# HaoruXue/spline-trajectory-optimization

Hardware: AMD Instinct MI355X
Metric: min-curvature QP solves/sec (N=2000 waypoints) (higher is better)
Workload: dtype f64

## Files before the change

### spline_trajectory_optimization_amd/csrc/rl_device.hpp

```cpp
#pragma once
#include <hip/hip_runtime.h>


namespace rl {

constexpr int kWave = 64;
constexpr int kMaxK = 5;

struct TrackDev {
  int k, n, nt, N;
  const double* t;
  const double* c0;
  const int* ell;
  const double* D;
  const int* sup;
  const double* base;
  const double* Ds;
  const double* base_s;
};

template <int K>
__device__ __forceinline__ void deboor(const double* __restrict__ t, double x, int l, int m,
                                       double (&h)[K + 1]) {
  double hh[K + 1];
// ... 321 lines not shown
__device__ __forceinline__ int stage_prefetch(const double2* ring, int nr, int nchunk, bool active, int hint, double2* stg, int lane) {
  const unsigned long long m = __ballot(active && hint >= 0 && hint < nr);
  const int first = m ? __ffsll((long long)m) - 1 : 0;
  const int lo = __builtin_amdgcn_readlane(window_start(hint, nchunk), first);
  const int base = m ? lo : 0;
  asm volatile("s_waitcnt lgkmcnt(0)" ::: "memory");
  stage_issue(ring, nr, base, stg, lane);
  return base;
}

template <bool ST = false, typename RingPtr>
__device__ __forceinline__ Hit search_ring_brute(RingPtr ring, int nr, double px, double py,
                                                 double dx, double dy) {
  Hit h{INFINITY, 0.0, kNoEdge};
  scan_edges<ST>(ring, nr, 0, nr, px, py, dx, dy, h);
  return h;
}


template <bool ST = false, typename RingPtr, typename CirclePtr>
__device__ __forceinline__ Hit search_ring_culled(RingPtr ring, int nr, CirclePtr circ, int nchunk,
                                                  double px, double py, double dx, double dy,
                                                  double dlen) {
  Hit h{INFINITY, 0.0, kNoEdge};
  for (int c = 0; c < nchunk; ++c) {
    const double mx = circ[3 * c] - px, my = circ[3 * c + 1] - py, r = circ[3 * c + 2];
    const double rr = r * dlen * (1.0 + 1e-9) + 1e-9;
    if (fabs(mx * dy - my * dx) > rr) continue;
    if (fabs(mx * dx + my * dy) > (dlen + r) * dlen * (1.0 + 1e-9) + 1e-9) continue;
    const int j0 = c * kChunk;
    scan_edges<ST>(ring, nr, j0, min(kChunk, nr - j0), px, py, dx, dy, h);
  }
  return h;
}

template <int CTRL, int ROW_MASK>
__device__ __forceinline__ double dpp_mov(double identity, double v) {
  int lo = __double2loint(v), hi = __double2hiint(v);
  lo = __builtin_amdgcn_update_dpp(__double2loint(identity), lo, CTRL, ROW_MASK, 0xf, false);
  hi = __builtin_amdgcn_update_dpp(__double2hiint(identity), hi, CTRL, ROW_MASK, 0xf, false);
  return __hiloint2double(hi, lo);
}
struct OpSum { static __device__ __forceinline__ double id() { return 0.0; }
               static __device__ __forceinline__ double f(double a, double b) { return a + b; } };
struct OpMax { static __device__ __forceinline__ double id() { return -INFINITY; }
               static __device__ __forceinline__ double f(double a, double b) { return fmax(a, b); } };
struct OpMin { static __device__ __forceinline__ double id() { return INFINITY; }
               static __device__ __forceinline__ double f(double a, double b) { return fmin(a, b); } };

template <typename Op>
__device__ __forceinline__ double wave_reduce(double v) {
  const double e = Op::id();
  v = Op::f(v, dpp_mov<0x111, 0xf>(e, v));
  v = Op::f(v, dpp_mov<0x112, 0xf>(e, v));
  v = Op::f(v, dpp_mov<0x114, 0xf>(e, v));
  v = Op::f(v, dpp_mov<0x118, 0xf>(e, v));
  v = Op::f(v, dpp_mov<0x142, 0xa>(e, v));
  v = Op::f(v, dpp_mov<0x143, 0xc>(e, v));
  const int lo = __builtin_amdgcn_readlane(__double2loint(v), 63);
  const int hi = __builtin_amdgcn_readlane(__double2hiint(v), 63);
  return __hiloint2double(hi, lo);
}
template <typename Op>
__device__ __forceinline__ double wave_reduce_bfly(double v) {
#define RL_BFLY(pattern)                                                                                        \
  {                                                                                                             \
    const int lo_ = __builtin_amdgcn_ds_swizzle(__double2loint(v), pattern);                                    \
    const int hi_ = __builtin_amdgcn_ds_swizzle(__double2hiint(v), pattern);                                    \
    v = Op::f(v, __hiloint2double(hi_, lo_));                                                                   \
  }
  RL_BFLY(0x041F) RL_BFLY(0x081F) RL_BFLY(0x101F) RL_BFLY(0x201F) RL_BFLY(0x401F)
#undef RL_BFLY
  const int other = (((int)threadIdx.x ^ 32) & 63) << 2;
  const int lo_ = __builtin_amdgcn_ds_bpermute(other, __double2loint(v));
  const int hi_ = __builtin_amdgcn_ds_bpermute(other, __double2hiint(v));
  return Op::f(v, __hiloint2double(hi_, lo_));
}
__device__ __forceinline__ double wave_max_bfly(double v) { return wave_reduce_bfly<OpMax>(v); }
__device__ __forceinline__ double wave_min_bfly(double v) { return wave_reduce_bfly<OpMin>(v); }
__device__ __forceinline__ double wave_sum(double v) { return wave_reduce<OpSum>(v); }
__device__ __forceinline__ double wave_max(double v) { return wave_reduce<OpMax>(v); }
__device__ __forceinline__ double wave_min(double v) { return wave_reduce<OpMin>(v); }

template <bool STAGED = false, bool ST = false, typename RingPtr, typename CirclePtr>
__device__ __forceinline__ Hit search_ring_windowed(RingPtr ring, int nr, CirclePtr circ,
                                                    CirclePtr sep, int nchunk, bool active, int hint,
                                                    double px, double py, double dx, double dy,
                                                    double dlen, const double* cmax, bool skip_guard = false,
                                                    unsigned long long* stamps = nullptr,
                                                    double2* stg = nullptr, int staged_base = -1) {
  const int lane = threadIdx.x & (kWave - 1);
  Hit h{INFINITY, 0.0, kNoEdge};
  const bool windowed = active && hint >= 0 && hint < nr;
  const int lo = window_start(hint, nchunk);
#ifdef RL_STAMPS
  unsigned long long w0 = 0, w1 = 0;
  asm volatile("s_memtime %0\n\ts_waitcnt lgkmcnt(0)" : "=s"(w0) :: "memory");
#endif
  if constexpr (!STAGED) {
    if (windowed) scan_window<kWinBatch, ST>(ring, nr, lo, lo, px, py, dx, dy, h, cmax);
  } else {
    bool todo = windowed;
    int base = staged_base;
    if (base >= 0) stage_wait();
    for (;;) {
      if (base >= 0) {
        int off = lo - base;
        if (off < 0) off += nr;
        if (todo && (off & (kChunk - 1)) == 0 && off + kWinEdges + 1 <= kStage) {
          scan_window<kStageBatch, ST>(StagedWindow{stg + stage_slot(off)}, nr, 0, lo, px, py, dx, dy, h, cmax, stamps);
          todo = false;
        }
      }
      const unsigned long long left = __ballot(todo);
      if (left == 0ull) break;
      base = __builtin_amdgcn_readlane(lo, __ffsll((long long)left) - 1);
      asm volatile("s_waitcnt lgkmcnt(0)" ::: "memory");
      stage_issue(reinterpret_cast<const double2*>(ring), nr, base, stg, lane);
      stage_wait();
    }
  }
#ifdef RL_STAMPS
  asm volatile("s_waitcnt vmcnt(0)\n\ts_memtime %0\n\ts_waitcnt lgkmcnt(0)" : "=s"(w1) :: "memory");
  if (stamps) stamps[0] += w1 - w0;
#endif
  if (skip_guard) return h;
  const bool found = h.best <= 1.0;
  const double di = active ? ((found ? h.best * dlen : dlen) * (1.0 + 1e-9) + 1e-9) : 0.0;
  auto chunk_in_window = [&](int c) {
    const int e0 = c * kChunk;
    const int cnt = min(kChunk, nr - e0);
    int off = e0 - lo;
    if (off < 0) off += nr;
    return off + cnt - 1 <= kWinEdges - 1;
  };
  bool slow = active;
  if (windowed && found && nchunk > 2 * kNear + 1) {
    const int ce = h.edge / kChunk;
    bool ok = sep[ce] > 2.0 * di;
    const bool centred = ce * kChunk == lo + kChunk && lo + kWinEdges <= nr;
    if (ok && !centred) {
#pragma unroll
      for (int u = -kNear; u <= kNear; ++u) {
        int c = ce + u;
        if (c < 0) c += nchunk;
        if (c >= nchunk) c -= nchunk;
        if (!chunk_in_window(c)) {
          const double mx = circ[3 * c] - px, my = circ[3 * c + 1] - py;
          const double lim = (di + circ[3 * c + 2]) * (1.0 + 1e-9);
          ok = ok && !(mx * mx + my * my <= lim * lim);
        }
      }
    }
    slow = !ok;
  }
  const unsigned long long sm = __ballot(slow);
  if (sm == 0ull) return h;
  const int first = __ffsll((long long)sm) - 1, last = 63 - __builtin_clzll(sm);
  auto bcast = [](double v, int src) {
    return __hiloint2double(__builtin_amdgcn_readlane(__double2hiint(v), src),
                            __builtin_amdgcn_readlane(__double2loint(v), src));
  };
  const double ccx = 0.5 * (bcast(px, first) + bcast(px, last));
  const double ccy = 0.5 * (bcast(py, first) + bcast(py, last));
  const double ex = px - ccx, ey = py - ccy;
  const double rho = wave_max(slow ? sqrt(ex * ex + ey * ey) + di : 0.0) * (1.0 + 1e-9);
  for (int c0 = 0; c0 < nchunk; c0 += kWave) {
    const int c = c0 + lane;
    bool pass = false;
    if (c < nchunk) {
      const double mx = circ[3 * c] - ccx, my = circ[3 * c + 1] - ccy;
      const double lim = rho + circ[3 * c + 2];
      pass = mx * mx + my * my <= lim * lim;
    }
    unsigned long long mask = __ballot(pass);
    while (mask) {
      const int cc = c0 + (__ffsll((long long)mask) - 1);
      mask &= mask - 1;
      const int e0 = cc * kChunk;
      const int cnt = min(kChunk, nr - e0);
      bool need = false;
      if (slow) {
        if (!(windowed && chunk_in_window(cc))) {
          const double mx = circ[3 * cc] - px, my = circ[3 * cc + 1] - py;
          const double lim = (di + circ[3 * cc + 2]) * (1.0 + 1e-9);
          need = mx * mx + my * my <= lim * lim;
        }
      }
      if (__any(need)) {
        Hit h2 = h;
        scan_edges_batched<kChunk, ST>(ring, nr, e0, cnt, px, py, dx, dy, h2);
        if (slow) h = h2;
      }
    }
  }
  return h;
}

}
```

### spline_trajectory_optimization_amd/csrc/rl_kernels.hpp

```cpp
#pragma once
#include "rl_device.hpp"
#include "rl_crmath.hpp"


namespace rl {

template <int K>
__global__ void k_build_tables(const double* __restrict__ t, int nt, const double* __restrict__ c0,
                               int N, int* __restrict__ ell, double* __restrict__ D,
                               double* __restrict__ base) {
  const int i = blockIdx.x * blockDim.x + threadIdx.x;
  if (i >= N) return;
  const int n = nt - K - 1;
  const double u = (double)i * (1.0 / (double)N);
  const int l = find_interval(t, K, n, u);
  ell[i] = l;
  double h[K + 1];
  double x = 0, y = 0, dx = 0, dy = 0;
#pragma unroll
  for (int m = 0; m < 3; ++m) {
    deboor<K>(t, u, l, m, h);
#pragma unroll
    for (int a = 0; a <= K; ++a) {
      D[((size_t)m * (K + 1) + a) * N + i] = h[a];
// ... 414 lines not shown
      const double denom = s2 * s2 * s2;
      double Pxx, Pxy, Pyy;
      cost_quotients(dTx, dTy, s2, denom, dTy * dTy, -2.0 * dTx * dTy, dTx * dTx, Pxx, Pxy, Pyy);
      double* tp = terms + tid;
      tp[0] = B2 * Pxx * B2;
      tp[kTermStrideA] = B2 * Pyy * B2;
      tp[2 * kTermStrideA] = Fx * Pxx * B2;
      tp[3 * kTermStrideA] = Fy * Pxy * B2;
      tp[4 * kTermStrideA] = Fy * Pyy * B2;
      tp[5 * kTermStrideA] = B2 * Pxy * Fx;
    }
    __syncthreads();
    if (wave == 0 && lane < 6) {
      const int cnt = min(kTermChunkA, M - ch * kTermChunkA);
      const double* tp = terms + lane * kTermStrideA;
      for (int u = 0; u < cnt; ++u) sacc += tp[u];
    }
    __syncthreads();
  }
  if (wave == 0) {
    auto lane_val = [&](int src) {
      return __hiloint2double(__builtin_amdgcn_readlane(__double2hiint(sacc), src), __builtin_amdgcn_readlane(__double2loint(sacc), src));
    };
    const double t0 = lane_val(0), t1 = lane_val(1), t2 = lane_val(2), t3 = lane_val(3), t4 = lane_val(4), t5 = lane_val(5);
    if (tid == 0) {
      H[4 * q + 0] = 2.0 * t0; H[4 * q + 1] = 0.0; H[4 * q + 2] = 0.0; H[4 * q + 3] = 2.0 * t1;
      g[2 * q + 0] = t2 + t2;
      g[2 * q + 1] = (t3 + t4) + (t5 + t4);
      if (Mout) Mout[q] = M;
    }
  }
}

template <int K>
__global__ void k_constraint_strict(TrackDev tr, const double* __restrict__ cx, const double* __restrict__ cy,
                                    const double* __restrict__ points, int idx, double* __restrict__ b,
                                    double* __restrict__ lba, double* __restrict__ uba) {
#pragma clang fp contract(off)
  const int s0 = tr.sup[2 * idx], s1 = tr.sup[2 * idx + 1];
  const double zx = cx[idx], zy = cy[idx];
  for (int i = s0 + blockIdx.x * blockDim.x + threadIdx.x; i < s1; i += gridDim.x * blockDim.x) {
    const int l = tr.ell[i];
    const double bi = tr.Ds[(size_t)(StrictRows<K>::D0 + idx - l + K) * tr.N + i];
    const double* p = points + (size_t)i * 19;
    const double nzx = p[0] - bi * zx, nzy = p[1] - bi * zy;
    const int r = i - s0;
    b[r] = bi;
    lba[2 * r] = fmin(p[9], p[11]) - nzx;
    lba[2 * r + 1] = fmin(p[10], p[12]) - nzy;
    uba[2 * r] = fmax(p[9], p[11]) - nzx;
    uba[2 * r + 1] = fmax(p[10], p[12]) - nzy;
  }
}

constexpr int kJointRowsPerThread = 3;

struct SweepArgs {
  TrackDev tr;
  int B;
  int form;
  const double* in;
  const double2* ringL;
  const double2* ringR;
  int nL, nR;
  int max_iter;
  int i_start[32];
  int search;
  double max_dist;
  double* out_ctrl;
  double* out_xy;
  double* out_points;
  int* n_success;
  int* status;
  double* gscratch;
  size_t gscratch_stride;
  double* dbg;
  int dbg_instances;
  int debug;
  int np_raise_at_start;
  double* aux;
  size_t aux_stride;
  int* n_raised;
  int* raise_flag;
};

#ifdef RL_STAMPS
#define RL_STAMP(var) do { __builtin_amdgcn_sched_barrier(0); asm volatile("s_memtime %0\n\ts_waitcnt lgkmcnt(0)" : "=s"(var) :: "memory"); __builtin_amdgcn_sched_barrier(0); } while (0)
#define RL_STAMP_ADD(slot, t1, t0) st_acc[slot] += (t1) - (t0)
#else
#define RL_STAMP(var) do { } while (0)
#define RL_STAMP_ADD(slot, t1, t0) do { } while (0)
#endif

#ifdef RL_ABLATION
#define RL_ABLATE(a, bit) (((a).debug & (bit)) != 0)
#else
#define RL_ABLATE(a, bit) false
#endif

struct SweepLds {
  int cpad, nLp, nRp, ncL, ncR;
  size_t off_cx, off_cy, off_red, off_sL, off_sR, off_rL, off_rR, off_cL, off_cR, off_pL, off_pR, off_hint, off_joint, off_stage,
         off_c12, off_terms, total;
};
constexpr int kSweepWaves = 4;
constexpr int kTermChunk = 256;
constexpr int kTermStride = kTermChunk + 2;
constexpr int kC12Doubles = 4 * (2 * kMaxK) + 8;
constexpr int kRedCoordMax = 194;

__host__ __device__ inline SweepLds sweep_lds_layout(int n, int N, int nL, int nR, bool rings_in_lds, bool sigma_in_lds,
                                                     bool joint = false, bool strict = false) {
  SweepLds L;
  L.cpad = (n + 1) & ~1;
  L.nLp = nL; L.nRp = nR;
  L.ncL = (nL + kChunk - 1) / kChunk;
  L.ncR = (nR + kChunk - 1) / kChunk;
  size_t o = 0;
  L.off_cx = o; o += L.cpad;
  L.off_cy = o; o += L.cpad;
  L.off_red = o; o += 8 * 24 + 4;
  L.off_cL = o; o += (size_t)((3 * L.ncL + 1) & ~1);
  L.off_cR = o; o += (size_t)((3 * L.ncR + 1) & ~1);
  L.off_pL = o; o += (size_t)((L.ncL + 1) & ~1);
  L.off_pR = o; o += (size_t)((L.ncR + 1) & ~1);
  L.off_joint = o; o += joint ? 128 + (size_t)((N + 15) / 16) * 2 : 0;
  L.off_hint = o; o += (size_t)(((size_t)2 * ((N + 3) & ~3) * sizeof(unsigned short) + 15) / 16) * 2;
  L.off_c12 = o; o += strict ? (joint ? (size_t)4 * L.cpad : kC12Doubles) : 0;
  L.off_sL = L.off_sR = L.off_rL = L.off_rR = 0;
  if (sigma_in_lds) {
    const size_t per = (size_t)((N + 1) & ~1) * (strict ? 2 : 1);
    L.off_sL = o; o += per;
    L.off_sR = o; o += per;
  }
  L.off_stage = 0;
  L.off_terms = 0;
  if (rings_in_lds) {
    L.off_rL = o; o += (size_t)2 * (nL + kRingPad);
    L.off_rR = o; o += (size_t)2 * (nR + kRingPad);
    if (strict) { L.off_terms = o; o += (size_t)6 * kTermStride; }
  } else {
    L.off_stage = o; o += (size_t)kSweepWaves * 2 * kStageSlots * 2;
    L.off_terms = L.off_stage;
    static_assert((size_t)kSweepWaves * 2 * kStageSlots * 2 >= (size_t)6 * kTermStride, "the cost terms fit the staged stretches");
  }
  L.total = o;
  return L;
}

constexpr int kSweepDumpHead = 16;

template <int K, int BLOCK, bool RINGS_LDS, bool JOINT = false, bool DUMP = false, bool SIGMA_LDS = RINGS_LDS, bool STRICT = false,
          bool RAISE = false, bool LITE = false>
__global__ __launch_bounds__(BLOCK, (BLOCK >= 512 || (!RINGS_LDS && !SIGMA_LDS && !JOINT)) ? 4 : 1) void k_sweep(SweepArgs a) {
  static_assert(!STRICT || (!DUMP && BLOCK == 256 && SIGMA_LDS == RINGS_LDS), "reference-order mode: the 256-thread kernels, all-LDS or all-global residency");
  static_assert(!(JOINT && (RAISE || LITE)), "the sliding-window driver exists in the fast and in the reference-order arithmetic");
  static_assert(!RAISE || STRICT, "numpy's error state is modelled in the reference-order mode");
  static_assert(!LITE || (STRICT && !RAISE), "the branch mode is a reduction of the reference-order kernel");
  if constexpr (RAISE) { if (!a.raise_flag || a.raise_flag[blockIdx.x] == 0) return; }
  extern __shared__ __attribute__((aligned(16))) unsigned char smem_raw[];
  double* smem = reinterpret_cast<double*>(smem_raw);
  const TrackDev& tr = a.tr;
  const int n = tr.n, N = tr.N;
  const int b = blockIdx.x;
  const int tid = threadIdx.x;
  const int lane = tid % kWave, wave = tid / kWave;
  constexpr int NW = BLOCK / kWave;
  const SweepLds L = sweep_lds_layout(n, N, a.nL, a.nR, RINGS_LDS, SIGMA_LDS, JOINT, STRICT);
  constexpr bool STAGED = !RINGS_LDS && BLOCK == 64 * kSweepWaves;
  double2* stgL = reinterpret_cast<double2*>(smem + L.off_stage) + (STAGED ? wave * 2 * kStageSlots : 0);
  double2* stgR = stgL + kStageSlots;
  double* cx = smem + L.off_cx;
  double* cy = smem + L.off_cy;
  double* red = smem + L.off_red;
  double* circL = smem + L.off_cL;
  double* circR = smem + L.off_cR;
  double* sepL = smem + L.off_pL;
  double* sepR = smem + L.off_pR;
  unsigned short* hints = reinterpret_cast<unsigned short*>(smem + L.off_hint);
  const int Npad = (N + 3) & ~3;
  double* sL; double* sR; double2* rL; double2* rR;
  {
    double* g = a.gscratch + (size_t)b * a.gscratch_stride;
    const size_t per_side = (size_t)((N + 1) & ~1) * (STRICT ? 2 : 1);
    if (SIGMA_LDS) { sL = smem + L.off_sL; sR = smem + L.off_sR; }
    else { sL = g; sR = sL + per_side; g = sR + per_side; }
    if (RINGS_LDS) {
      rL = reinterpret_cast<double2*>(smem + L.off_rL);
      rR = reinterpret_cast<double2*>(smem + L.off_rR);
    } else {
      if (RL_ABLATE(a, 8)) g = a.gscratch + (SIGMA_LDS ? 0 : 2 * per_side);
      rL = reinterpret_cast<double2*>(g);
      rR = rL + a.nL + kRingPad;
    }
  }
  const int nL = a.nL, nR = a.nR;
  double2* bL = reinterpret_cast<double2*>(sL);
  double2* bR = reinterpret_cast<double2*>(sR);
  const double* __restrict__ Ds = tr.Ds;
  using SR = StrictRows<K>;

  for (int j = tid; j < n; j += BLOCK) { cx[j] = tr.c0[j]; cy[j] = tr.c0[n + j]; }
  if (a.form == 1) {
    const double2* w = reinterpret_cast<const double2*>(a.in) + (size_t)b * N;
    for (int i = tid; i < N; i += BLOCK) {
      const double2 wi = w[i];
      if constexpr (STRICT) {
        const double* bs = tr.base_s;
        const double px = bs[i], py = bs[(size_t)N + i];
        rL[i] = make_double2(uf_madd(px, wi.x, bs[(size_t)2 * N + i]), uf_madd(py, wi.x, bs[(size_t)3 * N + i]));
        rR[i] = make_double2(uf_madd(px, wi.y, bs[(size_t)4 * N + i]), uf_madd(py, wi.y, bs[(size_t)5 * N + i]));
      } else {
        const double px = tr.base[i], py = tr.base[(size_t)N + i];
        const double nx = tr.base[(size_t)2 * N + i], ny = tr.base[(size_t)3 * N + i];
        rL[i] = make_double2(px + wi.x * nx, py + wi.x * ny);
        rR[i] = make_double2(px - wi.y * nx, py - wi.y * ny);
      }
    }
  } else if (a.form == 2) {
    const double4* w = reinterpret_cast<const double4*>(a.in) + (size_t)b * N;
    for (int i = tid; i < N; i += BLOCK) {
      const double4 wi = w[i];
      rL[i] = make_double2(wi.x, wi.y);
      rR[i] = make_double2(wi.z, wi.w);
    }
  } else {
    for (int i = tid; i < nL; i += BLOCK) rL[i] = a.ringL[i];
    for (int i = tid; i < nR; i += BLOCK) rR[i] = a.ringR[i];
  }
  __syncthreads();
  for (int q = tid; q < 2 * kRingPad; q += BLOCK) {
    if (q < kRingPad) rL[nL + q] = rL[q % nL]; else rR[nR + q - kRingPad] = rR[(q - kRingPad) % nR];
  }
  __syncthreads();
  if (a.search >= 1) {
    for (int c = tid; c < L.ncL + L.ncR; c += BLOCK) {
      const bool left = c < L.ncL;
      const int cc = left ? c : c - L.ncL;
      const double2* ring = left ? rL : rR;
      const int nr = left ? nL : nR;
      const int j0 = cc * kChunk, j1 = min(j0 + kChunk, nr);
      double xmin = INFINITY, xmax = -INFINITY, ymin = INFINITY, ymax = -INFINITY;
      for (int j = j0; j <= j1; ++j) {
        const double2 v = ring[j >= nr ? j - nr : j];
        xmin = fmin(xmin, v.x); xmax = fmax(xmax, v.x);
        ymin = fmin(ymin, v.y); ymax = fmax(ymax, v.y);
      }
      const double mx = 0.5 * (xmin + xmax), my = 0.5 * (ymin + ymax);
      double r2 = 0.0;
      for (int j = j0; j <= j1; ++j) {
        const double2 v = ring[j >= nr ? j - nr : j];
        const double ex = v.x - mx, ey = v.y - my;
        r2 = fmax(r2, ex * ex + ey * ey);
      }
      double* o = (left ? circL : circR) + 3 * cc;
      o[0] = mx; o[1] = my; o[2] = sqrt(r2) * (1.0 + 1e-12);
    }
    __syncthreads();
    if (a.search == 2) {
      for (int c = tid; c < L.ncL + L.ncR; c += BLOCK) {
        const bool left = c < L.ncL;
        const int cc = left ? c : c - L.ncL;
        const double* circ = left ? circL : circR;
        const int nc = left ? L.ncL : L.ncR;
        const double mx = circ[3 * cc], my = circ[3 * cc + 1], r = circ[3 * cc + 2];
        double gap = INFINITY;
        for (int q = 0; q < nc; ++q) {
          int dq = q - cc;
          if (dq < 0) dq = -dq;
          if (nc - dq < dq) dq = nc - dq;
          if (dq <= kNear) continue;
          const double ex = circ[3 * q] - mx, ey = circ[3 * q + 1] - my;
          gap = fmin(gap, sqrt(ex * ex + ey * ey) - r - circ[3 * q + 2]);
        }
        (left ? sepL : sepR)[cc] = gap * (1.0 - 1e-9) - 1e-9;
      }
      if (wave == 0) {
        double m = 0.0;
        for (int c = lane; c < L.ncL + L.ncR; c += kWave) {
          const double* o = c < L.ncL ? circL + 3 * c : circR + 3 * (c - L.ncL);
          const double v = fmax(fabs(o[0]), fabs(o[1])) + o[2];
          m = v <= 0x1p+1000 ? fmax(m, v) : INFINITY;
        }
        m = wave_max_bfly(m);
        if (lane == 0) red[kRedCoordMax] = m;
      }
      __syncthreads();
    }
  }

  double* jq = smem + L.off_joint;
  unsigned char* outside = reinterpret_cast<unsigned char*>(jq + 128);
  int* n_outside = reinterpret_cast<int*>(jq + 127);
  auto note_outside = [&](int i, double px, double py, double ndx, double ndy, double sl, double sr) {
    const double Lx = px + sl * ndx, Ly = py + sl * ndy;
    const double Rx = px + sr * (-ndx), Ry = py + sr * (-ndy);
    const bool out = fmin(Lx, Rx) > px || fmax(Lx, Rx) < px || fmin(Ly, Ry) > py || fmax(Ly, Ry) < py;
    const int was = outside[i];
    if ((int)out != was) { outside[i] = out ? 1 : 0; atomicAdd(n_outside, out ? 1 : -1); }
  };
  auto note_outside_pts = [&](int i, double px, double py, double2 Lp, double2 Rp) {
    const bool out = fmin(Lp.x, Rp.x) > px || fmax(Lp.x, Rp.x) < px || fmin(Lp.y, Rp.y) > py || fmax(Lp.y, Rp.y) < py;
    const int was = outside[i];
    if ((int)out != was) { outside[i] = out ? 1 : 0; atomicAdd(n_outside, out ? 1 : -1); }
  };
  if (JOINT) {
    for (int i = tid; i < N; i += BLOCK) outside[i] = 0;
    if (tid == 0) *n_outside = 0;
    __syncthreads();
  }

#ifdef RL_STAMPS
  unsigned long long st_cnt[4] = {0, 0, 0, 0};
#define RL_STRICT_COUNTS st_cnt
  unsigned long long st_fine[8] = {0, 0, 0, 0, 0, 0, 0, 0}, sf0 = 0, sf1 = 0;
#define RL_FSTAMP(slot) do { RL_STAMP(sf1); st_fine[slot] += sf1 - sf0; sf0 = sf1; } while (0)
#else
#define RL_STRICT_COUNTS nullptr
#define RL_FSTAMP(slot) do { } while (0)
#endif
  unsigned char* degen = (RAISE && a.aux) ? reinterpret_cast<unsigned char*>(a.aux + (size_t)b * a.aux_stride + 2 * L.cpad) : nullptr;
  int* n_degen = reinterpret_cast<int*>(red + 190);
  bool flag_mode = false;
  bool saw_degenerate = false;
  auto refresh = [&](int i0, int i1, int j0, int j1, int mode, int l_first = -1) {
    const int m0 = i1 - i0, m1 = j1 - j0, m = m0 + m1;
    const double* cmax = red + kRedCoordMax;
    if constexpr (STRICT) {
      int delta = 0;
      auto point = [&](int i, double& px, double& py, cr::Heading& hd, bool flags, auto&& in_heading) {
#pragma clang fp contract(off)
        const int l = tr.ell[i];
        double t0[K + 1], t1[K + 1];
        load_rows<K + 1>(t0, Ds + (size_t)SR::D0 * N, N, i);
        load_rows<K + 1>(t1, Ds + (size_t)SR::D1 * N, N, i);
        __builtin_amdgcn_sched_barrier(0);
        px = seq_dot_v<K + 1>(cx + (l - K), t0);
        py = seq_dot_v<K + 1>(cy + (l - K), t0);
        const double tx = seq_dot_v<K + 1>(cx + (l - K), t1);
        const double ty = seq_dot_v<K + 1>(cy + (l - K), t1);

        if constexpr (LITE && RL_LITE_NORMAL) {
          double nx, ny, inv_s2;
          scaled_normal(tx, ty, 1.0, nx, ny, inv_s2);
          hd.cl = nx; hd.sl = ny; hd.cr = -nx; hd.sr = -ny; hd.yaw = 0.0;
          return;
        }
        if (flags) {
          const double d2x = seq_dot<K + 1>(cx + (l - K), Ds + (size_t)SR::D2 * N, N, i);
          const double d2y = seq_dot<K + 1>(cy + (l - K), Ds + (size_t)SR::D2 * N, N, i);
          const double s2 = tx * tx + ty * ty;
          const double cross = fabs(tx * d2y - ty * d2x);
          const bool plainly_regular = cross >= 0x1p-200 && cross <= 0x1p+200 && s2 >= 0x1p-100 && s2 <= 0x1p+100;
          int now = 0;
          if (!__all(plainly_regular)) {
            const double den = sqrt(s2 * s2 * s2);
            const double curvature = cross / den;
            now = (den == 0.0 || !(curvature > 0.0) || !isfinite(curvature)) ? 1 : 0;
          }
          if constexpr (RAISE) { delta += now - (int)degen[i]; degen[i] = (unsigned char)now; }
          else if (now) saw_degenerate = true;
        }
#ifdef RL_STAMPS
        unsigned long long sh0, sh1;
        RL_STAMP(sh0);
#endif
        const bool sure = cr::heading_fast(tx, ty, hd, cr::kAtanTab, nullptr, in_heading);
        if (__any(!sure)) { if (!sure) hd = cr::heading(tx, ty); }
#ifdef RL_STAMPS
        RL_STAMP(sh1); st_fine[5] += sh1 - sh0; if (__any(!sure)) st_fine[6] += 1;
#endif
      };
      if (mode == 2) {
        const int nwt = (m + kWave - 1) / kWave;
        for (int wt = wave; wt < nwt; wt += NW) {
          const int r = wt * kWave + lane;
          const bool active = r < m;
          const int i = active ? (r < m0 ? i0 + r : j0 + (r - m0)) : (m0 > 0 ? i0 : j0);
          double px, py; cr::Heading hd;
#ifdef RL_STAMPS
          RL_STAMP(sf0);
#endif
          int baseL = -1, baseR = -1;
          point(i, px, py, hd, flag_mode && active, [&]() {
            if constexpr (STAGED) {
              baseL = stage_prefetch(reinterpret_cast<const double2*>(rL), nL, L.ncL, active, (int)hints[i], stgL, lane);
              baseR = stage_prefetch(reinterpret_cast<const double2*>(rR), nR, L.ncR, active, (int)hints[Npad + i], stgR, lane);
            }
          });
          RL_FSTAMP(0);
          const double dLx = a.max_dist * hd.cl, dLy = a.max_dist * hd.sl;
          const double dRx = a.max_dist * hd.cr, dRy = a.max_dist * hd.sr;
          const Hit hl = search_ring_windowed<STAGED, true>(rL, nL, circL, sepL, L.ncL, active, (int)hints[i], px, py,
                                                            dLx, dLy, a.max_dist, cmax, false, RL_STRICT_COUNTS, stgL, baseL);
          RL_FSTAMP(1);
          const Hit hr = search_ring_windowed<STAGED, true>(rR, nR, circR, sepR, L.ncR, active, (int)hints[Npad + i], px, py,
                                                            dRx, dRy, a.max_dist, cmax, false, RL_STRICT_COUNTS, stgR, baseR);
          RL_FSTAMP(2);
          if (active) {
            const double2 Lp = make_double2(uf_madd(px, hl.best_s, dLx), uf_madd(py, hl.best_s, dLy));
            const double2 Rp = make_double2(uf_madd(px, hr.best_s, dRx), uf_madd(py, hr.best_s, dRy));
            bL[i] = Lp; bR[i] = Rp;
            hints[i] = (unsigned short)(hl.edge == kNoEdge ? 0xFFFF : hl.edge);
            hints[Npad + i] = (unsigned short)(hr.edge == kNoEdge ? 0xFFFF : hr.edge);
            if (JOINT) note_outside_pts(i, px, py, Lp, Rp);
          }
        }
        if constexpr (RAISE) { if (delta != 0) atomicAdd(n_degen, delta); }
        return;
      }
      for (int task = tid; task < 2 * m; task += BLOCK) {
        const int side = task >= m;
        const int r = side ? task - m : task;
        const int i = r < m0 ? i0 + r : j0 + (r - m0);
        double px, py; cr::Heading hd;
        point(i, px, py, hd, flag_mode && side == 0, []() {});
        const double dx = a.max_dist * (side ? hd.cr : hd.cl), dy = a.max_dist * (side ? hd.sr : hd.sl);
        Hit h;
        if (mode == 1) {
          h = side ? search_ring_culled<true>(rR, nR, circR, L.ncR, px, py, dx, dy, a.max_dist)
                   : search_ring_culled<true>(rL, nL, circL, L.ncL, px, py, dx, dy, a.max_dist);
        } else {
          h = side ? search_ring_brute<true>(rR, nR, px, py, dx, dy) : search_ring_brute<true>(rL, nL, px, py, dx, dy);
        }
        (side ? bR : bL)[i] = make_double2(uf_madd(px, h.best_s, dx), uf_madd(py, h.best_s, dy));
        hints[side * Npad + i] = (unsigned short)(h.edge == kNoEdge ? 0xFFFF : h.edge);
      }
      if constexpr (RAISE) { if (delta != 0) atomicAdd(n_degen, delta); }
      if (JOINT) {
        __syncthreads();
        for (int r = tid; r < m; r += BLOCK) {
          const int i = r < m0 ? i0 + r : j0 + (r - m0);
          const int l = tr.ell[i];
          note_outside_pts(i, seq_dot<K + 1>(cx + (l - K), Ds + (size_t)SR::D0 * N, N, i),
                           seq_dot<K + 1>(cy + (l - K), Ds + (size_t)SR::D0 * N, N, i), bL[i], bR[i]);
        }
      }
      return;
    }
    if (mode == 2) {
      const int nwt = (m + kWave - 1) / kWave;
#ifndef RL_SWEEP_TASKS
#define RL_SWEEP_TASKS 1
#endif
      if constexpr (BLOCK >= 512 && !JOINT && RL_SWEEP_TASKS) {
        for (int tk = wave; tk < 2 * nwt; tk += NW) {
          const int wt = tk >> 1;
          const bool right = tk & 1;
          const int r = wt * kWave + lane;
          const bool active = r < m;
          const int i = active ? (r < m0 ? i0 + r : j0 + (r - m0)) : (m0 > 0 ? i0 : j0);
          CurvePoint<K, 1> c;
          eval_sample<K, 1>(tr, cx, cy, i, tr.ell[i], c);
          double dx, dy, inv_s2;
          scaled_normal(c.dx, c.dy, a.max_dist, dx, dy, inv_s2);
          if (!right) {
            const Hit hl = search_ring_windowed(rL, nL, circL, sepL, L.ncL, active, (int)hints[i], c.x, c.y, dx, dy, a.max_dist, cmax, false);
            if (active) { sL[i] = hl.best_s; hints[i] = (unsigned short)(hl.edge == kNoEdge ? 0xFFFF : hl.edge); }
          } else {
            const Hit hr = search_ring_windowed(rR, nR, circR, sepR, L.ncR, active, (int)hints[Npad + i], c.x, c.y, -dx, -dy, a.max_dist, cmax, false);
            if (active) { sR[i] = hr.best_s; hints[Npad + i] = (unsigned short)(hr.edge == kNoEdge ? 0xFFFF : hr.edge); }
          }
        }
        return;
      }
      for (int wt = wave; wt < nwt; wt += NW) {
        const int r = wt * kWave + lane;
        const bool active = r < m;
        const int i = active ? (r < m0 ? i0 + r : j0 + (r - m0)) : (m0 > 0 ? i0 : j0);
        const int l = (l_first >= 0 && wt == wave && r < m0) ? l_first : tr.ell[i];
#ifdef RL_STAMPS
        RL_STAMP(sf0);
#endif
        int baseL = -1, baseR = -1;
        if constexpr (STAGED) {
          baseL = stage_prefetch(reinterpret_cast<const double2*>(rL), nL, L.ncL, active, (int)hints[i], stgL, lane);
          baseR = stage_prefetch(reinterpret_cast<const double2*>(rR), nR, L.ncR, active, (int)hints[Npad + i], stgR, lane);
        }
        CurvePoint<K, 1> c;
        eval_sample<K, 1>(tr, cx, cy, i, l, c);
        double dx, dy, inv_s2;
        scaled_normal(c.dx, c.dy, a.max_dist, dx, dy, inv_s2);
        RL_FSTAMP(0);
        const bool skip = RL_ABLATE(a, 2);
#ifdef RL_STAMPS
        unsigned long long ws[2] = {0, 0};
        const Hit hl = search_ring_windowed<STAGED>(rL, nL, circL, sepL, L.ncL, active, (int)hints[i], c.x, c.y,
                                                    dx, dy, a.max_dist, cmax, skip, ws, stgL, baseL);
// ... 1525 lines not shown
```

### spline_trajectory_optimization_amd/csrc/rl_mincurv.hip

```cpp
#include "../../include/rl_mincurv.h"

#include <hip/hip_runtime.h>

#include <algorithm>
#include <cmath>
#include <cstdio>
#include <cstdlib>
#include <cstring>
#include <mutex>
#include <string>
#include <vector>

#include "rl_kernels.hpp"
#include "rl_qss_df.hpp"
#include "rl_global.hpp"
#include "rl_global2.hpp"
#include "rl_global_xy.hpp"
#include "rl_dtrack.hpp"
#include "rl_mintime.hpp"
#include "rl_bicycle.hpp"
#include "rl_region.hpp"

namespace {

// ... 730 lines not shown
      while (b0 < N && (double)b0 * step < te) ++b0;
      if (b0 - a0 > widest) widest = b0 - a0;
    }
    if (widest > rl::kJointRowsPerThread * 256)
      return fail(RL_ERR_UNSUPPORTED, "sliding-window variant: a window spans more than 768 samples");
  }
  int arith = ctx->arith;
  if (!ctx->arith_explicit && arith == RL_ARITH_REFERENCE && (k != 5 || g_dbg_instances > 0)) arith = RL_ARITH_FAST;
  const bool lite = arith == RL_ARITH_BRANCH;
  const bool strict = arith == RL_ARITH_REFERENCE || lite;
  if (strict) {
    if (joint && lite) return fail(RL_ERR_UNSUPPORTED, "the branch arithmetic (rl_ctx_set_arith) covers run_min_curvature_qp; the sliding-window driver exists in the fast and in the reference-order arithmetic");
    RL_HIP(hipSetDevice(ctx->device));
    if (int rc = ensure_strict_tables(ctx, trk)) return rc;
  }
  rl::SweepArgs a;
  std::memset(&a, 0, sizeof(a));
  a.tr = trk->dev();
  a.B = B;
  a.form = form;
  a.in = in_dev;
  if (form == RL_BOUNDS_SHARED_RINGS) {
    if (trk->nL == 0) return fail(RL_ERR_ARG, "rl_track_set_rings was not called");
    a.ringL = reinterpret_cast<const double2*>(trk->ringL.p);
    a.ringR = reinterpret_cast<const double2*>(trk->ringR.p);
    a.nL = trk->nL; a.nR = trk->nR;
  } else if (form == RL_BOUNDS_WIDTHS || form == RL_BOUNDS_POINTS) {
    if (!in_dev) return fail(RL_ERR_ARG, "bounds input is null");
    a.nL = N; a.nR = N;
  } else {
    return fail(RL_ERR_ARG, "bad bounds_form");
  }
  a.max_iter = max_iter;
  for (int j = 0; j < max_iter; ++j) a.i_start[j] = i_start[j];
  a.search = search;
  a.max_dist = 100.0;
#ifdef RL_ABLATION
  if (const char* dbg = getenv("RL_DEBUG_FLAGS")) a.debug = atoi(dbg);
#endif
#ifdef RL_STAMPS
  const bool dbg_ok = true;
#else
  const bool dbg_ok = !strict;
#endif
  if (g_dbg_instances > 0 && (joint || k == 5) && dbg_ok) {
    const int ninst = std::min(g_dbg_instances, B);
    size_t need = joint ? (size_t)max_iter * (size_t)(i_max - i_min) * (48 + 9 * rl::kJointRowsPerThread * 256 + 2 * n)
                        : (size_t)ninst * max_iter * 2 * (size_t)(i_max - i_min) * (rl::kSweepDumpHead + 2 * n);
#ifdef RL_STAMPS
    need = std::max(need, (size_t)B * 4 * 16);
#endif
    a.dbg_instances = ninst;
    if (g_dbg_len < need) {
      if (g_dbg_buf) (void)hipFree(g_dbg_buf);
      RL_HIP(hipMalloc(reinterpret_cast<void**>(&g_dbg_buf), need * sizeof(double)));
      g_dbg_len = need;
    }
    RL_HIP(hipMemsetAsync(g_dbg_buf, 0, need * sizeof(double), ctx->stream));
    a.dbg = g_dbg_buf;
  }
  a.out_ctrl = out_ctrl; a.out_xy = out_xy; a.out_points = out_points;
  a.n_success = n_success; a.status = status;
  RL_HIP(hipSetDevice(ctx->device));
  SweepPlan p = plan_sweep(ctx, n, N, a.nL, a.nR, B, joint, strict);
  if (p.lds_bytes > (size_t)ctx->max_lds) return fail(RL_ERR_UNSUPPORTED, "problem does not fit LDS");
  if (p.sigma_in_lds && !p.rings_in_lds && (joint || k != 5 || a.dbg)) {
    p.sigma_in_lds = false;
    p.lds_bytes = rl::sweep_lds_layout(n, N, a.nL, a.nR, false, false, joint).total * sizeof(double);
    p.gscratch_doubles += (size_t)2 * ((N + 1) & ~1);
  }
  if (p.gscratch_doubles) {
    const size_t need = p.gscratch_doubles * (size_t)B;
    if (trk->gscratch.n < need) RL_HIP(trk->gscratch.alloc(need));
    a.gscratch = trk->gscratch.p;
    a.gscratch_stride = p.gscratch_doubles;
  }
  if (strict && !lite) {
    const size_t per = (size_t)2 * ((n + 1) & ~1) + (size_t)2 * ((N + 15) / 16) + (size_t)2 * N;
    const size_t flags = ((size_t)B + 1) / 2;
    if (trk->aux.n < per * (size_t)B + flags) RL_HIP(trk->aux.alloc(per * (size_t)B + flags));
    a.aux = trk->aux.p;
    a.aux_stride = per;
    a.np_raise_at_start = ctx->np_raise_at_start;
    a.raise_flag = reinterpret_cast<int*>(trk->aux.p + per * (size_t)B);
    RL_HIP(hipMemsetAsync(a.raise_flag, 0, (size_t)B * sizeof(int), ctx->stream));
  }
  if (stats) {
    stats->lds_bytes = (int)p.lds_bytes;
    stats->block_threads = p.block;
    stats->rings_in_lds = p.rings_in_lds ? 1 : (p.sigma_in_lds ? 2 : 0);
    stats->reserved[0] = arith;
  }
  if (plan_out) *plan_out = p;
  return launch_sweep(ctx, k, p, a, joint, strict, lite);
}

int rl_mincurv_solve_batch_dev(rl_ctx* ctx, const rl_track* trk, int bounds_form, const double* in,
                               int B, const int* i_start, int max_iter, int search,
                               double* out_ctrl, double* out_xy, int* n_success, int* status,
                               rl_stats* stats) {
  if (!out_xy) return fail(RL_ERR_ARG, "out_xy is null");
  return solve_batch_common(ctx, trk, bounds_form, in, B, i_start, max_iter, search, out_ctrl, out_xy,
                            nullptr, n_success, status, stats, nullptr);
}

int rl_mincurv_solve_batch_host(rl_ctx* ctx, const rl_track* trk, int bounds_form, const double* in,
                                int B, const int* i_start, int max_iter, int search,
                                double* out_ctrl, double* out_xy, int* n_success, int* status,
                                rl_stats* stats) {
  if (!ctx || !trk || !out_ctrl || !out_xy) return fail(RL_ERR_ARG, "null argument");
  if (B <= 0) return fail(RL_ERR_ARG, "B <= 0");
  RL_HIP(hipSetDevice(ctx->device));
  const int n = trk->n, N = trk->N;
  const int cols = bounds_form == RL_BOUNDS_WIDTHS ? 2 : (bounds_form == RL_BOUNDS_POINTS ? 4 : 0);
  PoolBuf<double> din(ctx), dctrl(ctx), dxy(ctx);
  PoolBuf<int> dns(ctx), dst(ctx);
  if (cols) {
    if (!in) return fail(RL_ERR_ARG, "bounds input is null");
    RL_HIP(din.alloc((size_t)B * N * cols));
    RL_HIP(hipMemcpyAsync(din.p, in, din.n * sizeof(double), hipMemcpyHostToDevice, ctx->stream));
  }
  RL_HIP(dctrl.alloc((size_t)B * n * 2)); RL_HIP(dxy.alloc((size_t)B * N * 2));
  RL_HIP(dns.alloc((size_t)B * 2 * (max_iter > 0 ? max_iter : 1))); RL_HIP(dst.alloc(B));
  RL_HIP(hipEventRecord(ctx->ev0, ctx->stream));
  int rc = solve_batch_common(ctx, trk, bounds_form, din.p, B, i_start, max_iter, search, dctrl.p, dxy.p,
                              nullptr, dns.p, dst.p, stats, nullptr);
  if (rc) return rc;
  RL_HIP(hipEventRecord(ctx->ev1, ctx->stream));
  RL_HIP(hipMemcpyAsync(out_ctrl, dctrl.p, dctrl.n * sizeof(double), hipMemcpyDeviceToHost, ctx->stream));
  RL_HIP(hipMemcpyAsync(out_xy, dxy.p, dxy.n * sizeof(double), hipMemcpyDeviceToHost, ctx->stream));
  if (n_success) RL_HIP(hipMemcpyAsync(n_success, dns.p, (size_t)B * 2 * max_iter * sizeof(int), hipMemcpyDeviceToHost, ctx->stream));
  if (status) RL_HIP(hipMemcpyAsync(status, dst.p, (size_t)B * sizeof(int), hipMemcpyDeviceToHost, ctx->stream));
  RL_HIP(hipStreamSynchronize(ctx->stream));
  if (stats) {
    float ms = 0.f;
    RL_HIP(hipEventElapsedTime(&ms, ctx->ev0, ctx->ev1));
    stats->kernel_ms = ms;
  }
  return RL_OK;
}

extern "C++" {
namespace {

int host_find_interval(const std::vector<double>& t, int k, int n, double x) {
  int lo = k, hi = n - 1;
  while (lo < hi) {
    const int mid = (lo + hi + 1) >> 1;
    if (x >= t[mid]) lo = mid; else hi = mid - 1;
  }
  return lo;
}

int global_tables(const rl_ctx* ctx, const rl_track* trk) {
  if (trk->gq_valid) return RL_OK;
  const int k = trk->k, n = trk->n, N = trk->N, np = n - k;
  if (np < 2 * (k + 1)) return fail(RL_ERR_UNSUPPORTED, "too few control points for the global QP");
  if (np > rl::kGMaxNp) return fail(RL_ERR_UNSUPPORTED, "global QP: more than 192 free control points");
  if (N >= (1 << 24)) return fail(RL_ERR_UNSUPPORTED, "global QP: N too large");
  std::vector<int> rows(np, 0);
  const double step = 1.0 / (double)N;
  for (int i = 0; i < N; ++i) ++rows[host_find_interval(trk->t_host, k, n, (double)i * step) - k];
  auto partition = [&](int R, std::vector<int>& chunk, std::vector<int>& span) {
    chunk.clear(); span.assign(np + 1, 0);
    int row = 0;
    for (int s = 0; s < np; ++s) {
// ... 913 lines not shown
```

Baseline: 102,100.

## Balance strict refresh wave tiles by splitting left/right ring searches across waves

In the strict mode-2 refresh sweep, when the number of wave tiles leaves 1 or 2 leftover tiles for 4 waves, the leftover tiles' left and right ring searches are split across idle waves. Heading data passes through a small LDS hand-off buffer behind a block barrier, and joint outside-point bookkeeping is redone afterwards. This targets tail imbalance, where one wave does both searches while the others sit idle. Separately, the per-chunk separation bounds are stored as round-down floats to shrink LDS use. The cost is extra barriers and position recomputation, and the path is on by default with an env override.

```diff
diff --git a/spline_trajectory_optimization_amd/csrc/rl_device.hpp b/spline_trajectory_optimization_amd/csrc/rl_device.hpp
--- a/spline_trajectory_optimization_amd/csrc/rl_device.hpp
+++ b/spline_trajectory_optimization_amd/csrc/rl_device.hpp
@@ -427,9 +427,9 @@
 __device__ __forceinline__ double wave_max(double v) { return wave_reduce<OpMax>(v); }
 __device__ __forceinline__ double wave_min(double v) { return wave_reduce<OpMin>(v); }
 
-template <bool STAGED = false, bool ST = false, typename RingPtr, typename CirclePtr>
+template <bool STAGED = false, bool ST = false, typename RingPtr, typename CirclePtr, typename SepPtr>
 __device__ __forceinline__ Hit search_ring_windowed(RingPtr ring, int nr, CirclePtr circ,
-                                                    CirclePtr sep, int nchunk, bool active, int hint,
+                                                    SepPtr sep, int nchunk, bool active, int hint,
                                                     double px, double py, double dx, double dy,
                                                     double dlen, const double* cmax, bool skip_guard = false,
                                                     unsigned long long* stamps = nullptr,
@@ -482,7 +482,7 @@
   bool slow = active;
   if (windowed && found && nchunk > 2 * kNear + 1) {
     const int ce = h.edge / kChunk;
-    bool ok = sep[ce] > 2.0 * di;
+    bool ok = (double)sep[ce] > 2.0 * di;
     const bool centred = ce * kChunk == lo + kChunk && lo + kWinEdges <= nr;
     if (ok && !centred) {
 #pragma unroll
diff --git a/spline_trajectory_optimization_amd/csrc/rl_kernels.hpp b/spline_trajectory_optimization_amd/csrc/rl_kernels.hpp
--- a/spline_trajectory_optimization_amd/csrc/rl_kernels.hpp
+++ b/spline_trajectory_optimization_amd/csrc/rl_kernels.hpp
@@ -520,6 +520,7 @@
   size_t aux_stride;
   int* n_raised;
   int* raise_flag;
+  int balance;
 };
 
 #ifdef RL_STAMPS
@@ -539,9 +540,12 @@
 struct SweepLds {
   int cpad, nLp, nRp, ncL, ncR;
   size_t off_cx, off_cy, off_red, off_sL, off_sR, off_rL, off_rR, off_cL, off_cR, off_pL, off_pR, off_hint, off_joint, off_stage,
-         off_c12, off_terms, total;
+         off_c12, off_terms, off_hand, total;
 };
 constexpr int kSweepWaves = 4;
+constexpr int kHandSlots = 2;
+__host__ __device__ constexpr int refresh_moves(int T) { return (T & 3) == 1 ? 1 : (T & 3) == 2 ? 2 : 0; }
+__host__ __device__ constexpr int refresh_receiver(int T, int w) { return (T & 3) == 1 ? 1 : 2 + w; }
 constexpr int kTermChunk = 256;
 constexpr int kTermStride = kTermChunk + 2;
 constexpr int kC12Doubles = 4 * (2 * kMaxK) + 8;
@@ -560,11 +564,12 @@
   L.off_red = o; o += 8 * 24 + 4;
   L.off_cL = o; o += (size_t)((3 * L.ncL + 1) & ~1);
   L.off_cR = o; o += (size_t)((3 * L.ncR + 1) & ~1);
-  L.off_pL = o; o += (size_t)((L.ncL + 1) & ~1);
-  L.off_pR = o; o += (size_t)((L.ncR + 1) & ~1);
+  L.off_pL = o; o += (size_t)((L.ncL + 3) / 4) * 2;
+  L.off_pR = o; o += (size_t)((L.ncR + 3) / 4) * 2;
   L.off_joint = o; o += joint ? 128 + (size_t)((N + 15) / 16) * 2 : 0;
   L.off_hint = o; o += (size_t)(((size_t)2 * ((N + 3) & ~3) * sizeof(unsigned short) + 15) / 16) * 2;
   L.off_c12 = o; o += strict ? (joint ? (size_t)4 * L.cpad : kC12Doubles) : 0;
+  L.off_hand = o; o += strict ? (size_t)kHandSlots * kWave * 2 : 0;
   L.off_sL = L.off_sR = L.off_rL = L.off_rR = 0;
   if (sigma_in_lds) {
     const size_t per = (size_t)((N + 1) & ~1) * (strict ? 2 : 1);
@@ -613,8 +618,8 @@
   double* red = smem + L.off_red;
   double* circL = smem + L.off_cL;
   double* circR = smem + L.off_cR;
-  double* sepL = smem + L.off_pL;
-  double* sepR = smem + L.off_pR;
+  float* sepL = reinterpret_cast<float*>(smem + L.off_pL);
+  float* sepR = reinterpret_cast<float*>(smem + L.off_pR);
   unsigned short* hints = reinterpret_cast<unsigned short*>(smem + L.off_hint);
   const int Npad = (N + 3) & ~3;
   double* sL; double* sR; double2* rL; double2* rR;
@@ -711,7 +716,7 @@
           const double ex = circ[3 * q] - mx, ey = circ[3 * q + 1] - my;
           gap = fmin(gap, sqrt(ex * ex + ey * ey) - r - circ[3 * q + 2]);
         }
-        (left ? sepL : sepR)[cc] = gap * (1.0 - 1e-9) - 1e-9;
+        (left ? sepL : sepR)[cc] = __double2float_rd(gap * (1.0 - 1e-9) - 1e-9);
       }
       if (wave == 0) {
         double m = 0.0;
@@ -766,6 +771,13 @@
     const double* cmax = red + kRedCoordMax;
     if constexpr (STRICT) {
       int delta = 0;
+      auto position = [&](int i, double& px, double& py) {
+        const int l = tr.ell[i];
+        double t0[K + 1];
+        load_rows<K + 1>(t0, Ds + (size_t)SR::D0 * N, N, i);
+        px = seq_dot_v<K + 1>(cx + (l - K), t0);
+        py = seq_dot_v<K + 1>(cy + (l - K), t0);
+      };
       auto point = [&](int i, double& px, double& py, cr::Heading& hd, bool flags, auto&& in_heading) {
 #pragma clang fp contract(off)
         const int l = tr.ell[i];
@@ -811,37 +823,69 @@
       };
       if (mode == 2) {
         const int nwt = (m + kWave - 1) / kWave;
-        for (int wt = wave; wt < nwt; wt += NW) {
+        const int moves = a.balance ? refresh_moves(nwt) : 0;
+        double2* hand = reinterpret_cast<double2*>(smem + L.off_hand);
+        int src = -1;
+        for (int w = 0; w < moves; ++w) src = refresh_receiver(nwt, w) == wave ? w : src;
+        const bool mover = wave < moves, receiver = src >= 0;
+        for (int pass = moves ? -1 : 0;; ++pass) {
+          const bool split = pass < 0;
+          const int wt = split ? nwt - moves + (mover ? wave : src) : wave + pass * NW;
+          if (!split && wt >= nwt - moves) break;
+          const bool doL = !split || mover, doR = !split || receiver;
           const int r = wt * kWave + lane;
-          const bool active = r < m;
+          const bool active = (doL || doR) && r < m;
           const int i = active ? (r < m0 ? i0 + r : j0 + (r - m0)) : (m0 > 0 ? i0 : j0);
-          double px, py; cr::Heading hd;
+          double px = 0.0, py = 0.0; cr::Heading hd{};
 #ifdef RL_STAMPS
           RL_STAMP(sf0);
 #endif
           int baseL = -1, baseR = -1;
-          point(i, px, py, hd, flag_mode && active, [&]() {
-            if constexpr (STAGED) {
-              baseL = stage_prefetch(reinterpret_cast<const double2*>(rL), nL, L.ncL, active, (int)hints[i], stgL, lane);
-              baseR = stage_prefetch(reinterpret_cast<const double2*>(rR), nR, L.ncR, active, (int)hints[Npad + i], stgR, lane);
-            }
-          });
+          if (doL) {
+            point(i, px, py, hd, flag_mode && active, [&]() {
+              if constexpr (STAGED) {
+                baseL = stage_prefetch(reinterpret_cast<const double2*>(rL), nL, L.ncL, active, (int)hints[i], stgL, lane);
+                baseR = stage_prefetch(reinterpret_cast<const double2*>(rR), nR, L.ncR, active, (int)hints[Npad + i], stgR, lane);
+              }
+            });
+          } else if (doR) {
+            if constexpr (STAGED) baseR = stage_prefetch(reinterpret_cast<const double2*>(rR), nR, L.ncR, active, (int)hints[Npad + i], stgR, lane);
+            position(i, px, py);
+          }
+          if (split) {
+            if (mover) hand[wave * kWave + lane] = make_double2(hd.cr, hd.sr);
+            if constexpr (RINGS_LDS) __syncthreads(); else lds_barrier();
+            if (receiver) { const double2 d = hand[src * kWave + lane]; hd.cr = d.x; hd.sr = d.y; }
+          }
           RL_FSTAMP(0);
           const double dLx = a.max_dist * hd.cl, dLy = a.max_dist * hd.sl;
           const double dRx = a.max_dist * hd.cr, dRy = a.max_dist * hd.sr;
-          const Hit hl = search_ring_windowed<STAGED, true>(rL, nL, circL, sepL, L.ncL, active, (int)hints[i], px, py,
-                                                            dLx, dLy, a.max_dist, cmax, false, RL_STRICT_COUNTS, stgL, baseL);
+          Hit hl{INFINITY, 0.0, kNoEdge}, hr{INFINITY, 0.0, kNoEdge};
+          if (doL) hl = search_ring_windowed<STAGED, true>(rL, nL, circL, sepL, L.ncL, active, (int)hints[i], px, py,
+                                                           dLx, dLy, a.max_dist, cmax, false, RL_STRICT_COUNTS, stgL, baseL);
           RL_FSTAMP(1);
-          const Hit hr = search_ring_windowed<STAGED, true>(rR, nR, circR, sepR, L.ncR, active, (int)hints[Npad + i], px, py,
-                                                            dRx, dRy, a.max_dist, cmax, false, RL_STRICT_COUNTS, stgR, baseR);
+          if (doR) hr = search_ring_windowed<STAGED, true>(rR, nR, circR, sepR, L.ncR, active, (int)hints[Npad + i], px, py,
+                                                           dRx, dRy, a.max_dist, cmax, false, RL_STRICT_COUNTS, stgR, baseR);
           RL_FSTAMP(2);
           if (active) {
             const double2 Lp = make_double2(uf_madd(px, hl.best_s, dLx), uf_madd(py, hl.best_s, dLy));
             const double2 Rp = make_double2(uf_madd(px, hr.best_s, dRx), uf_madd(py, hr.best_s, dRy));
-            bL[i] = Lp; bR[i] = Rp;
-            hints[i] = (unsigned short)(hl.edge == kNoEdge ? 0xFFFF : hl.edge);
-            hints[Npad + i] = (unsigned short)(hr.edge == kNoEdge ? 0xFFFF : hr.edge);
-            if (JOINT) note_outside_pts(i, px, py, Lp, Rp);
+            if (doL) { bL[i] = Lp; hints[i] = (unsigned short)(hl.edge == kNoEdge ? 0xFFFF : hl.edge); }
+            if (doR) { bR[i] = Rp; hints[Npad + i] = (unsigned short)(hr.edge == kNoEdge ? 0xFFFF : hr.edge); }
+            if (JOINT && doL && doR) note_outside_pts(i, px, py, Lp, Rp);
+          }
+        }
+        if (JOINT && moves) {
+          __syncthreads();
+          for (int w = 0; w < moves; ++w) {
+            if (refresh_receiver(nwt, w) != wave) continue;
+            const int r = (nwt - moves + w) * kWave + lane;
+            if (r < m) {
+              const int i = r < m0 ? i0 + r : j0 + (r - m0);
+              double px, py;
+              position(i, px, py);
+              note_outside_pts(i, px, py, bL[i], bR[i]);
+            }
           }
         }
         if constexpr (RAISE) { if (delta != 0) atomicAdd(n_degen, delta); }
diff --git a/spline_trajectory_optimization_amd/csrc/rl_mincurv.hip b/spline_trajectory_optimization_amd/csrc/rl_mincurv.hip
--- a/spline_trajectory_optimization_amd/csrc/rl_mincurv.hip
+++ b/spline_trajectory_optimization_amd/csrc/rl_mincurv.hip
@@ -836,6 +836,8 @@
     a.aux = trk->aux.p;
     a.aux_stride = per;
     a.np_raise_at_start = ctx->np_raise_at_start;
+    a.balance = 1;
+    if (const char* f = getenv("RL_REFRESH_BALANCE")) if (f[0] == '0' || f[0] == '1') a.balance = f[0] - '0';
     a.raise_flag = reinterpret_cast<int*>(trk->aux.p + per * (size_t)B);
     RL_HIP(hipMemsetAsync(a.raise_flag, 0, (size_t)B * sizeof(int), ctx->stream));
   }
```

After: 101,700 (median of 2 runs). No clear change (-0.3%).
